# alexfrom0815/IR-BPP

Measured on AMD Instinct MI355X. Metric: env steps/sec (placements/sec) across N parallel bins, higher is better.
Workload: dtype f64

## Files before the change

### irbpp_amd/csrc/irbpp_kernels.hip

```cpp
#include <hip/hip_runtime.h>
#include <math.h>
#include <stdint.h>

#include "contours_device.h"
#include "irbpp_device.h"
#include "../../include/irbpp.h"

#ifndef IRBPP_PASS
#define IRBPP_PASS 1
#endif

#undef IRBPP_HERE
#undef IRBPP_PASS_NS
#if IRBPP_PASS == 1
#define IRBPP_HERE ::irbpp::
#elif IRBPP_PASS == 2
#define IRBPP_HERE ::irbpp::wg512::
#define IRBPP_PASS_NS wg512
#else
#define IRBPP_HERE ::irbpp::wg128::
#define IRBPP_PASS_NS wg128
#endif

namespace irbpp {
// ... 1295 lines not shown
                    khi[l] = ah; klo[l] = al; kps[l] = (uint16_t)ap;
                }
            }
            const int j_next = j > 1 ? (j >> 1) : k;
            if (j >= 128 || j_next >= 128 || (j == 1 && k == npad)) __syncthreads();
            else IRBPP_WAVE_SYNC();
        }
    for (int r = tid; r < want; r += BLOCK) out[r] = sel[kps[r]];
    __syncthreads();
}

#ifdef IRBPP_AB_EMIT_ACCOUNT
#define IRBPP_EMIT_STAMP(k) do { if (io.phase_cycles && threadIdx.x == 0) io.phase_cycles[(size_t)b * PHASE_ROW + (k)] = (long long)clock64(); } while (0)
#else
#define IRBPP_EMIT_STAMP(k) do {} while (0)
#endif
__device__ inline void emit_observation(const Params& P, const State& S, const StepIO& io, const Lds& L, int b, int item,
                                        int nvalid, float* obs, const double* zsrc, const uint32_t* gvalid, uint32_t amap) {
    const int tid = threadIdx.x;
    const int R = P.R, AC = P.AC, Ax = P.Ax, Ay = P.Ay;
    const int X = fdiv(tid, Ay, P.mg_ay), Y = tid - X * Ay;
    const int prev_rows = io.obs_rows != nullptr ? io.obs_rows[b] : -1;
    if (tid == 0) ((unsigned long long*)L.redd)[7] = ~0ull;
    uint32_t* keys = (uint32_t*)L.scratch;
    uint32_t* okey = keys + R * AC;
    uint32_t* hist = (uint32_t*)L.img;
    int n = 0;
    if (tid < 64) {
        const int lane = tid, cx = lane & 15;
        for (int r0 = 0; r0 < R; r0 += 4) {
            const int r = r0 + (lane >> 4);
            uint32_t col = 0u;
            if (r < R && cx < Ay) {
                const uint32_t* const vrow = L.vmask + ((amap >> (4 * r)) & 15u) * 16;
#pragma unroll
                for (int cy = 0; cy < 16; ++cy) col |= ((vrow[cy] >> cx) & 1u) << cy;
                col &= (1u << Ax) - 1u;
            }
            const int cnt = __popc(col), incl = wave_inclusive_sum(cnt);
            int at = n + incl - cnt;
            while (col != 0u) {
                const int cy = __ffs((int)col) - 1;
                col &= col - 1u;
                keys[at++] = ((uint32_t)r << 16) | ((uint32_t)cy << 8) | (uint32_t)cx;
            }
            n += __builtin_amdgcn_readlane(incl, 63);
        }
        if (tid == 0) L.redi[34] = n;
    }
    __syncthreads();
    n = L.redi[34];
    IRBPP_EMIT_STAMP(11);
    int nrows;
    bool fallback = false;
    const uint32_t* rows;
    if (n > 0 && n <= P.S) {
        nrows = n;
        rows = keys;
    } else if (n > P.S) {
        select_smallest(P, L, zsrc, nullptr, n, P.S, [&](int e) { return keys[e]; }, okey, keys, hist);
        nrows = P.S;
        rows = okey;
        __syncthreads();
    } else {
        fallback = true;
        const int total_cells = R * AC;
        const int want = total_cells < P.S ? total_cells : P.S;
        auto cell_key = [&](int e) {
            const int r = fdiv(e, AC, P.mg_ac), c = e - r * AC, x = fdiv(c, Ay, P.mg_ay);
            return ((uint32_t)r << 16) | ((uint32_t)x << 8) | (uint32_t)(c - x * Ay);
        };
        if (nvalid == 0) {
            for (int e = tid; e < want; e += BLOCK) okey[e] = cell_key(e);
            __syncthreads();
        } else {
            select_smallest(P, L, zsrc, gvalid, total_cells, want, cell_key, okey, keys, hist);
        }
        nrows = total_cells < P.S ? total_cells : P.S;
        rows = okey;
        __syncthreads();
    }

    IRBPP_EMIT_STAMP(12);
    int write_rows = P.S;
    if (io.obs_rows != nullptr) {
        if (prev_rows >= 0) write_rows = prev_rows > nrows ? prev_rows : nrows;
        if (tid == 0) io.obs_rows[b] = nrows;
    }
    float best = INFINITY;
    int bi = 0x7fffffff;
    for (int rep = 0; rep < IRBPP_REPS(3); ++rep)
    for (int row = tid; row < write_rows; row += BLOCK) {
        float v0 = 0.0f, v1 = 0.0f, v2 = 0.0f, v3 = 0.0f, v4 = 0.0f;
        if (row < nrows) {
            const uint32_t k = rows[row];
            float rv;
            if (fallback) rv = (float)((gvalid[(k >> 16) * 16 + ((k >> 8) & 255u)] >> (k & 255u)) & 1u);
            else rv = (float)zsrc[(k >> 16) * AC + ((k >> 8) & 255u) * Ay + (k & 255u)];
            v0 = (float)(k >> 16);
            v1 = (float)((k >> 8) & 255u);
            v2 = (float)(k & 255u);
            v3 = fallback ? (float)P.bin_z : rv;
            v4 = fallback ? rv : 1.0f;
            S.cand[(size_t)b * P.S + row] = k;
            if (!fallback && rv < best) { best = rv; bi = row; }
        }
        float* const o = obs + 5 * row;
        o[0] = v0; o[1] = v1; o[2] = v2; o[3] = v3; o[4] = v4;
    }
    IRBPP_EMIT_STAMP(13);
    if (tid == 0) {
        S.bs[b].cur_item = item;
        S.bs[b].nvalid = nvalid;
        S.bs[b].nrows = nrows;
    }
    if (io.auto_action != nullptr) {
        {
#define IRBPP_ARGMIN_STEP(CTRL, ROWS)                                                                                          \
            {                                                                                                                  \
                const float ob = __int_as_float(__builtin_amdgcn_update_dpp(__float_as_int(best), __float_as_int(best), CTRL, ROWS, 0xF, false)); \
                const int oi = __builtin_amdgcn_update_dpp(bi, bi, CTRL, ROWS, 0xF, false);                                     \
                if (ob < best || (ob == best && oi < bi)) { best = ob; bi = oi; }                                               \
            }
            IRBPP_ARGMIN_STEP(0x111, 0xF) IRBPP_ARGMIN_STEP(0x112, 0xF) IRBPP_ARGMIN_STEP(0x114, 0xF) IRBPP_ARGMIN_STEP(0x118, 0xF)
            IRBPP_ARGMIN_STEP(0x142, 0xA) IRBPP_ARGMIN_STEP(0x143, 0xC)
#undef IRBPP_ARGMIN_STEP
        }
        if ((tid & 63) == 63) {
            const uint32_t fb = (uint32_t)__float_as_int(best + 0.0f);
            const uint32_t su = fb ^ ((fb >> 31) != 0u ? 0xFFFFFFFFu : 0x80000000u);
            atomicMin((unsigned long long*)L.redd + 7, ((unsigned long long)su << 32) | (uint32_t)bi);
        }
        __syncthreads();
        if (tid == 0) {
            const int won = (int)(uint32_t)(((const unsigned long long*)L.redd)[7] & 0xFFFFFFFFull);
            io.auto_action[b] = won == 0x7fffffff ? 0 : won;
        }
    }
    stamp(io, b, 4);
}

#endif
template <int IPT>
__device__ inline void split_handover(const Params& P, const State& S, const Lds& L, int b, int slot, int item, int nvalid) {
    const int tid = threadIdx.x;
    const KernArgsPtr ka = cold_args();
    constexpr int IMGS = IPT * (BLOCK / 16);
    constexpr int CLIST = CONTOUR_CLIST;
    uint16_t* const rows = (uint16_t*)L.scratch;
    uint16_t* const cwords = rows + IMGS * 16;
    uint16_t* const clist = L.clist;
    {
        uint32_t* gb = ka->S.w_valid + (size_t)b * P.R * 16;
        for (int rep = 0; rep < IRBPP_REPS(14); ++rep)
#pragma unroll 1
        for (int i = tid; i < P.R * 16; i += BLOCK) gb[i] = L.vbits[i];
        __syncthreads();
    }
    int ntasks = 0;
    for (int rep = 0; rep < IRBPP_REPS(9); ++rep) { if (rep) __syncthreads(); ntasks = IRBPP_HERE contour_tasks(P, L); }
    int ncand = 0, niso = 0;
    uint32_t* gi = (uint32_t*)(ka->S.w_img + (size_t)b * P.wimg * 16);
    uint8_t* gr = ka->S.w_imgrot + (size_t)b * P.wimg;
    const int xcd = (int)(__builtin_amdgcn_s_getreg((31 << 11) | 20) & (NXCD - 1));
    for (int base = 0; base < ntasks; base += IMGS) {
        int batch_total = 0;
        for (int rep = 0; rep < IRBPP_REPS(9); ++rep) {
            IRBPP_HERE contour_images<IPT>(P, L, rows, base, false);
            batch_total = IRBPP_HERE contour_candidates<IPT>(P, L, rows, base, ntasks, cwords);
        }
        niso += batch_total >> 16;
        batch_total &= 0xFFFF;
        const int nb = ntasks - base < IMGS ? ntasks - base : IMGS;
        const uint32_t* lr = (const uint32_t*)rows;
        for (int rep = 0; rep < IRBPP_REPS(14); ++rep) {
#pragma unroll 1
        for (int i = tid; i < nb * 8; i += BLOCK) gi[(size_t)base * 8 + i] = lr[i];
#pragma unroll 1
        for (int i = tid; i < nb; i += BLOCK) gr[base + i] = (uint8_t)(L.tasklist[base + i] >> 8);
        }
        const int nsub = batch_total <= CLIST ? 1 : IMGS;
        for (int sub = 0; sub < nsub; ++sub) {
            int total = 0;
            for (int rep = 0; rep < IRBPP_REPS(10); ++rep) total = IRBPP_HERE contour_list<IPT>(L, rows, clist, base, ntasks, nsub, sub, cwords);
            if (tid == 0) {
                int at = -1, seg = xcd;
                if (total > 0) {
                    for (int k = 0; k < NXCD && at < 0; ++k) {
                        seg = (xcd + k) & (NXCD - 1);
                        const int got = atomicAdd(ka->S.w_total + seg * XCD_STRIDE, total);
                        if (got + total <= P.seg_cap) at = got;
                        else atomicSub(ka->S.w_total + seg * XCD_STRIDE, total);
                    }
                    if (at < 0) raise_error(S, IRBPP_DEVERR_CAPACITY);
                }
                L.redi[11] = at;
                L.redi[12] = seg;
            }
            __syncthreads();
            if (L.redi[11] >= 0) {
                uint2* flat = ka->S.w_cand + (size_t)L.redi[12] * P.seg_cap + L.redi[11];
#pragma unroll 1
                for (int i = tid; i < total; i += BLOCK) {
                    const uint32_t e = clist[i];
                    flat[i] = make_uint2((uint32_t)b, ((uint32_t)(base + (e & 127u)) << 8) | (((e >> 11) & 15u) << 4) | ((e >> 7) & 15u));
                }
            }
            ncand += total;
        }
        __syncthreads();
    }
    uint32_t* gv = ka->S.w_vmask + (size_t)b * P.R * 16;
    for (int rep = 0; rep < IRBPP_REPS(14); ++rep)
#pragma unroll 1
    for (int i = tid; i < P.R * 16; i += BLOCK) gv[i] = L.vmask[i];
    if (tid == 0) {
        int32_t* m = ka->S.w_meta + (size_t)b * WMETA;
        m[0] = ntasks;
        m[1] = ncand;
        m[2] = nvalid;
        m[3] = item;
        m[5] = (int32_t)alias_map(L, P.R, item);
        int heavy = 0;
        const int turn = ka->io.heavy_turn;
        if (turn >= 0 && ncand + niso >= P.heavy_thr) {
            int32_t* hv = ka->S.w_heavy + (size_t)turn * (XCD_STRIDE + P.heavy_cap);
            const int pos = atomicAdd(hv, 1);
            if (pos < P.heavy_cap) { hv[XCD_STRIDE + pos] = b; heavy = 1; }
        }
        m[4] = heavy;
    }
}

#if IRBPP_PASS == 1
template <bool HEAVY_FIRST, int SPEC>
__device__ __forceinline__ void emit_body(const Params& P_run, const Tables& T, const State& S, const StepIO& io, const int mode, unsigned char* smem) {
    Params P_spec;
    const Params& P = SPEC == 0 ? P_run : (P_spec = specialise<SPEC>(P_run), P_spec);
    Lds L = {};
    L.vmask = (uint32_t*)(smem + P.e_vmask);
    L.redd = (double*)(smem + P.e_red);
    L.redi = (int*)(L.redd + 8);
    L.img = (uint16_t*)(smem + P.e_hist);
    L.scratch = smem + P.e_keys;
    const bool some = mode == MODE_RESET && io.bin_list != nullptr;
    const int tid = threadIdx.x;
    if (blockIdx.x == 0 && tid < NXCD) { S.w_total[tid * XCD_STRIDE] = 0; S.w_nround[tid * XCD_STRIDE] = 0; }
    if (blockIdx.x == 0 && tid == 0 && io.err_out != nullptr) *io.err_out = *S.err;
#ifdef IRBPP_AB_EMIT_ACCOUNT
    const long long t_entry = (long long)clock64();
#endif
    int slot = (int)blockIdx.x + io.block_off, b = 0;
    bool mapped = false;
    if constexpr (HEAVY_FIRST) {
        const int hg = io.heavy_turn >= 0 ? P.heavy_cap : 0;
        if ((int)blockIdx.x < hg) {
            const int32_t* hv = S.w_heavy + (size_t)io.heavy_turn * (XCD_STRIDE + P.heavy_cap);
            if (blockIdx.x == 0 && tid == 0) S.w_heavy[(size_t)(io.heavy_turn ^ 1) * (XCD_STRIDE + P.heavy_cap)] = 0;
            int cnt = hv[0];
            cnt = cnt < P.heavy_cap ? cnt : P.heavy_cap;
            if ((int)blockIdx.x >= cnt) return;
            b = hv[XCD_STRIDE + blockIdx.x];
            slot = b;
            mapped = true;
        } else {
            slot -= hg;
        }
    }
    if (!mapped) {
        b = ((mode == MODE_STEP || mode == MODE_CANDS) && io.use_order) ? S.order[slot] : some ? io.bin_list[slot] : slot;
        if constexpr (HEAVY_FIRST)
            if (io.heavy_turn >= 0 && b >= 0 && b < P.N && S.w_meta[(size_t)b * WMETA + 4] != 0) return;
    }
    if (b < 0 || b >= P.N) return;
#ifdef IRBPP_AB_EMIT_ACCOUNT
    if (io.phase_cycles && tid == 0) { io.phase_cycles[(size_t)b * PHASE_ROW + 6] = t_entry; io.phase_cycles[(size_t)b * PHASE_ROW + 7] = (long long)clock64(); }
#endif
    float* obs = io.obs + (size_t)(some ? slot : b) * io.obs_stride;
    const uint32_t* gv = S.w_vmask + (size_t)b * P.R * 16;
#pragma unroll 1
    for (int i = tid; i < P.R * 16; i += BLOCK) L.vmask[i] = gv[i];
    const int nvalid = S.w_meta[(size_t)b * WMETA + 2], item = S.w_meta[(size_t)b * WMETA + 3];
    const uint32_t amap = (uint32_t)S.w_meta[(size_t)b * WMETA + 5];
    __syncthreads();
    stamp(io, b, 3);
    emit_observation(P, S, io, L, b, item, nvalid, obs, S.w_posz + (size_t)b * P.R * P.AC, S.w_valid + (size_t)b * P.R * 16, amap);
    IRBPP_EMIT_STAMP(14);
}
#define IRBPP_EMIT_KERNEL(NAME, HF, SPEC)                                                                                \
    extern "C" __global__ void __launch_bounds__(BLOCK) __attribute__((amdgpu_waves_per_eu(8, 8)))                      \
    NAME(const Params P, const Tables T, const State S, const StepIO io, const int mode) {                              \
        extern __shared__ __attribute__((aligned(16))) unsigned char smem[];                                            \
        emit_body<HF, SPEC>(P, T, S, io, mode, smem);                                                                   \
    }
IRBPP_EMIT_KERNEL(irbpp_emit_kernel, true, 0)
#ifndef IRBPP_NO_SPEC
IRBPP_EMIT_KERNEL(irbpp_emit_kernel_s1, true, 1)
IRBPP_EMIT_KERNEL(irbpp_emit_kernel_s2, true, 2)
IRBPP_EMIT_KERNEL(irbpp_emit_kernel_s3, true, 3)
IRBPP_EMIT_KERNEL(irbpp_emit_kernel_s4, true, 4)
IRBPP_EMIT_KERNEL(irbpp_emit_kernel_s5, true, 5)
#endif

template <int SPEC>
__device__ __forceinline__ void emit_wave_body(const Params& P_run, const Tables& T, const State& S, const StepIO& io, const int mode,
                                               unsigned char* smem) {
    Params P_spec;
    const Params& P = SPEC == 0 ? P_run : (P_spec = specialise<SPEC>(P_run), P_spec);
    int* const need = (int*)(smem + P.e_need);
    const int tid = threadIdx.x, lane = tid & 63, wave = __builtin_amdgcn_readfirstlane(tid >> 6);
    const int R = P.R, AC = P.AC, Ax = P.Ax, Ay = P.Ay;
    const bool some = mode == MODE_RESET && io.bin_list != nullptr;
    if (blockIdx.x == 0 && tid < NXCD) { S.w_total[tid * XCD_STRIDE] = 0; S.w_nround[tid * XCD_STRIDE] = 0; }
    if (blockIdx.x == 0 && tid == 0 && io.err_out != nullptr) *io.err_out = *S.err;
    const int local = (int)blockIdx.x * WAVES + wave;
    const int slot = local + io.block_off;
    int b = -1;
    if (local < io.n_slots) b = ((mode == MODE_STEP || mode == MODE_CANDS) && io.use_order) ? S.order[slot] : some ? io.bin_list[slot] : slot;
    if (b >= P.N) b = -1;
    b = __builtin_amdgcn_readfirstlane(b);
    if (lane == 0) need[wave] = -1;
    if (b >= 0) {
        uint32_t* const vm = (uint32_t*)(smem + wave * P.ew_bytes);
        uint32_t* const keys = vm + R * 16;
        const uint32_t* gv = S.w_vmask + (size_t)b * R * 16;
        for (int i = lane; i < R * 16; i += 64) vm[i] = gv[i];
        const int nvalid = S.w_meta[(size_t)b * WMETA + 2], item = S.w_meta[(size_t)b * WMETA + 3];
        const uint32_t amap = (uint32_t)S.w_meta[(size_t)b * WMETA + 5];
        const int prev_rows = io.obs_rows != nullptr ? io.obs_rows[b] : -1;
        float* const obs = io.obs + (size_t)(some ? slot : b) * io.obs_stride;
        const double* const zsrc = S.w_posz + (size_t)b * R * AC;
        const uint32_t* const gvalid = S.w_valid + (size_t)b * R * 16;
        stamp(io, b, 3, lane == 0);
        IRBPP_WAVE_SYNC();
        const int cx = lane & 15;
        auto column = [&](int r) {
            uint32_t col = 0u;
            if (r < R && cx < Ay) {
                const uint32_t* const vrow = vm + ((amap >> (4 * r)) & 15u) * 16;
#pragma unroll
                for (int cy = 0; cy < 16; ++cy) col |= ((vrow[cy] >> cx) & 1u) << cy;
                col &= (1u << Ax) - 1u;
            }
            return col;
        };
        int n = 0;
#pragma unroll 1
        for (int r0 = 0; r0 < R; r0 += 4) n += __builtin_amdgcn_readlane(wave_inclusive_sum(__popc(column(r0 + (lane >> 4)))), 63);
        if (n > P.S || (n == 0 && nvalid > 0)) {
            if (lane == 0) need[wave] = b;
        } else {
            int at0 = 0;
#pragma unroll 1
            for (int r0 = 0; r0 < R; r0 += 4) {
                const int r = r0 + (lane >> 4);
                uint32_t col = column(r);
                const int cnt = __popc(col), incl = wave_inclusive_sum(cnt);
                int at = at0 + incl - cnt;
                while (col != 0u) {
                    const int cy = __ffs((int)col) - 1;
                    col &= col - 1u;
                    keys[at++] = ((uint32_t)r << 16) | ((uint32_t)cy << 8) | (uint32_t)cx;
                }
                at0 += __builtin_amdgcn_readlane(incl, 63);
            }
            IRBPP_WAVE_SYNC();
            const bool fallback = n == 0;
            const int total_cells = R * AC;
            const int nrows = fallback ? (total_cells < P.S ? total_cells : P.S) : n;
            int write_rows = P.S;
            if (io.obs_rows != nullptr) {
                if (prev_rows >= 0) write_rows = prev_rows > nrows ? prev_rows : nrows;
                if (lane == 0) io.obs_rows[b] = nrows;
            }
            float best = INFINITY;
            int bi = 0x7fffffff;
            for (int row = lane; row < write_rows; row += 64) {
                float v0 = 0.0f, v1 = 0.0f, v2 = 0.0f, v3 = 0.0f, v4 = 0.0f;
                if (row < nrows) {
                    uint32_t k;
                    if (fallback) {
                        const int r = fdiv(row, AC, P.mg_ac), c = row - r * AC, x = fdiv(c, Ay, P.mg_ay);
                        k = ((uint32_t)r << 16) | ((uint32_t)x << 8) | (uint32_t)(c - x * Ay);
                    } else {
                        k = keys[row];
                    }
                    float rv;
                    if (fallback) rv = (float)((gvalid[(k >> 16) * 16 + ((k >> 8) & 255u)] >> (k & 255u)) & 1u);
                    else rv = (float)zsrc[(k >> 16) * AC + ((k >> 8) & 255u) * Ay + (k & 255u)];
                    v0 = (float)(k >> 16);
                    v1 = (float)((k >> 8) & 255u);
                    v2 = (float)(k & 255u);
                    v3 = fallback ? (float)P.bin_z : rv;
                    v4 = fallback ? rv : 1.0f;
                    S.cand[(size_t)b * P.S + row] = k;
                    if (!fallback && rv < best) { best = rv; bi = row; }
                }
                float* const o = obs + 5 * row;
                o[0] = v0; o[1] = v1; o[2] = v2; o[3] = v3; o[4] = v4;
            }
            if (lane == 0) {
                S.bs[b].cur_item = item;
                S.bs[b].nvalid = nvalid;
                S.bs[b].nrows = nrows;
            }
            if (io.auto_action != nullptr) {
#define IRBPP_ARGMIN_STEP(CTRL, ROWS)                                                                                          \
                {                                                                                                              \
                    const float ob = __int_as_float(__builtin_amdgcn_update_dpp(__float_as_int(best), __float_as_int(best), CTRL, ROWS, 0xF, false)); \
                    const int oi = __builtin_amdgcn_update_dpp(bi, bi, CTRL, ROWS, 0xF, false);                                 \
                    if (ob < best || (ob == best && oi < bi)) { best = ob; bi = oi; }                                           \
                }
                IRBPP_ARGMIN_STEP(0x111, 0xF) IRBPP_ARGMIN_STEP(0x112, 0xF) IRBPP_ARGMIN_STEP(0x114, 0xF) IRBPP_ARGMIN_STEP(0x118, 0xF)
                IRBPP_ARGMIN_STEP(0x142, 0xA) IRBPP_ARGMIN_STEP(0x143, 0xC)
#undef IRBPP_ARGMIN_STEP
                if (lane == 63) io.auto_action[b] = bi == 0x7fffffff ? 0 : bi;
            }
            stamp(io, b, 4, lane == 0);
        }
    }
    __syncthreads();
    if ((need[0] & need[1] & need[2] & need[3]) == -1) return;
    Lds L = {};
    L.vmask = (uint32_t*)(smem + P.e_vmask);
    L.redd = (double*)(smem + P.e_red);
    L.redi = (int*)(L.redd + 8);
    L.img = (uint16_t*)(smem + P.e_hist);
    L.scratch = smem + P.e_keys;
#pragma unroll 1
    for (int w = 0; w < WAVES; ++w) {
        const int bw = __builtin_amdgcn_readfirstlane(need[w]);
        if (bw < 0) continue;
        const int slot_w = (int)blockIdx.x * WAVES + w + io.block_off;
        float* const obs = io.obs + (size_t)(some ? slot_w : bw) * io.obs_stride;
        const uint32_t* gv = S.w_vmask + (size_t)bw * R * 16;
        __syncthreads();
#pragma unroll 1
        for (int i = tid; i < R * 16; i += BLOCK) L.vmask[i] = gv[i];
        const int nvalid = S.w_meta[(size_t)bw * WMETA + 2], item = S.w_meta[(size_t)bw * WMETA + 3];
        const uint32_t amap_w = (uint32_t)S.w_meta[(size_t)bw * WMETA + 5];
        __syncthreads();
        stamp(io, bw, 3);
        emit_observation(P, S, io, L, bw, item, nvalid, obs, S.w_posz + (size_t)bw * R * AC, S.w_valid + (size_t)bw * R * 16, amap_w);
    }
}
#define IRBPP_EMIT_WAVE_KERNEL(NAME, SPEC)                                                                                  \
    extern "C" __global__ void __launch_bounds__(BLOCK) __attribute__((amdgpu_waves_per_eu(8, 8)))                      \
    NAME(const Params P, const Tables T, const State S, const StepIO io, const int mode) {                              \
        extern __shared__ __attribute__((aligned(16))) unsigned char smem[];                                            \
        emit_wave_body<SPEC>(P, T, S, io, mode, smem);                                                                  \
    }
IRBPP_EMIT_WAVE_KERNEL(irbpp_emit_wave_kernel, 0)
#ifndef IRBPP_NO_SPEC
IRBPP_EMIT_WAVE_KERNEL(irbpp_emit_wave_kernel_s1, 1)
IRBPP_EMIT_WAVE_KERNEL(irbpp_emit_wave_kernel_s2, 2)
IRBPP_EMIT_WAVE_KERNEL(irbpp_emit_wave_kernel_s5, 5)
#endif

#ifndef IRBPP_TRACE_SHORT
#define IRBPP_TRACE_SHORT 0
#endif
constexpr int TRACE_P = IRBPP_TRACE_P;
constexpr int TRACE_CAP = 128;
constexpr int TRACE_LDS_CAP = 56, TRACE_SLOT = TRACE_LDS_CAP + 4;
constexpr int TRACE_SPILL = TRACE_CAP - TRACE_LDS_CAP;
constexpr int TRACE_SHORT = IRBPP_TRACE_SHORT;
static_assert(TRACE_CAP <= 64 * TRACE_P, "a border must fit one polygon round");
static_assert(ROUND_POINTS == 64 * TRACE_P, "a round record holds one polygon round");
constexpr int TRACE_BIG = 768;
constexpr int TRACE_FSTRIDE = FRAME_WORDS;
static_assert(TRACE_FSTRIDE % 2 == 1 && (TRACE_SLOT / 4) % 2 == 1 && TRACE_SLOT % 4 == 0, "odd dword strides in LDS");
constexpr int TRACE_BIG_BYTES = 6 * TRACE_BIG + 64;
constexpr int TRACE_WAVE_BYTES = TRACE_BIG_BYTES + 64 * TRACE_SPILL;
template <int TRACE_CPW>
__device__ __forceinline__ void trace_body(const Params& P, const State& S, long long* prof) {
    constexpr int SLOT = TRACE_SLOT, CAP = TRACE_CAP, LCAP = TRACE_LDS_CAP, PP = TRACE_P;
    __shared__ __attribute__((aligned(16))) uint8_t slots[TRACE_CPW * SLOT];
    __shared__ __attribute__((aligned(16))) uint32_t sfr[TRACE_CPW * TRACE_FSTRIDE];
    __shared__ uint32_t dps[64 * PP];
    __shared__ uint8_t dpscratch[64 * PP];
    const int lane = threadIdx.x;
    const int seg_cap = P.seg_cap;
    int seg_n[NXCD], seg_first[NXCD + 1];
    seg_first[0] = 0;
#pragma unroll
    for (int s = 0; s < NXCD; ++s) {
        const int n = S.w_total[s * XCD_STRIDE];
        seg_n[s] = n < seg_cap ? n : seg_cap;
        seg_first[s + 1] = seg_first[s] + (seg_n[s] + TRACE_CPW - 1) / TRACE_CPW;
    }
    for (int chunk = blockIdx.x; chunk < seg_first[NXCD]; chunk += gridDim.x) {
        const long long t_start = prof ? (long long)clock64() : 0;
        int seg = 0;
#pragma unroll
        for (int s = 1; s < NXCD; ++s) seg += chunk >= seg_first[s] ? 1 : 0;
        int first_chunk = 0, count = 0;
#pragma unroll
        for (int s = 0; s < NXCD; ++s) if (s == seg) { first_chunk = seg_first[s]; count = seg_n[s]; }
        const int gi = (chunk - first_chunk) * TRACE_CPW + lane;
        const bool have = lane < TRACE_CPW && gi < count;
        const size_t g = (size_t)seg * seg_cap + gi;
        int my_n = 0, rk = 0, x0 = 0, y0 = 0;
        uint32_t* const fr = sfr + (lane < TRACE_CPW ? lane : 0) * TRACE_FSTRIDE;
        uint8_t* const my_slot = slots + (lane < TRACE_CPW ? lane : 0) * SLOT;
        uint8_t* const wave_spill = S.w_big + (size_t)blockIdx.x * TRACE_WAVE_BYTES + TRACE_BIG_BYTES;
        if (have) {
            const uint2 ce = S.w_cand[g];
            const uint32_t e = ce.y;
            const int b = (int)ce.x, img = (int)((e >> 8) & 511u);
            x0 = e & 15u;
            y0 = (e >> 4) & 15u;
            rk = b * P.R + (int)S.w_imgrot[(size_t)b * P.wimg + img];
            const uint4* gi = (const uint4*)(S.w_img + ((size_t)b * P.wimg + img) * 16);
            const uint4 v0 = gi[0], v1 = gi[1];
            const uint32_t w[8] = {v0.x, v0.y, v0.z, v0.w, v1.x, v1.y, v1.z, v1.w};
            uint32_t r[16], c[16];
#pragma unroll
            for (int q = 0; q < 8; ++q) {
                r[2 * q] = c[2 * q] = w[q] & 0xFFFFu;
                r[2 * q + 1] = c[2 * q + 1] = w[q] >> 16;
            }
            transpose16(c);
            frames_store(fr, r, c);
        }
        const long long t_staged = prof ? (long long)clock64() : 0;
        {
            const int n = trace_border_fast(fr, x0, y0, my_slot, LCAP, have, wave_spill + lane * TRACE_SPILL, TRACE_SPILL);
            if (n < 0) { if (lane == 0) atomicOr(S.err, IRBPP_DEVERR_TRACE_GUARD); }
            else my_n = n;
        }
        {
            unsigned long long big = __ballot(my_n > CAP);
            while (big != 0ull) {
                const int l0 = __ffsll((long long)big) - 1;
                big &= big - 1ull;
                if (lane == l0) {
                    uint8_t* gsc = S.w_big + (size_t)blockIdx.x * TRACE_WAVE_BYTES;
                    SlotMem m;
                    m.pts = gsc; m.dst = gsc + TRACE_BIG; m.stk = (uint32_t*)(gsc + 2 * TRACE_BIG); m.cap = TRACE_BIG; m.cap_stk = TRACE_BIG;
                    uint16_t* im = (uint16_t*)(gsc + 6 * TRACE_BIG);
                    for (int q = 0; q < 16; ++q) { im[q] = (uint16_t)frame_raw_row(fr, q); im[16 + q] = (uint16_t)frame_raw_col(fr, q); }
                    if (contour_vertices(im, im + 16, x0, y0, m, S.w_vmask + (size_t)rk * 16) != 0)
                        atomicOr(S.err, IRBPP_DEVERR_TRACE_GUARD);
                    my_n = 0;
                }
            }
        }
        const bool spilled = __ballot(my_n > LCAP) != 0ull;
        if (spilled) {
            __builtin_amdgcn_fence(__ATOMIC_RELEASE, "workgroup");
            __builtin_amdgcn_fence(__ATOMIC_ACQUIRE, "workgroup");
        }
        const long long t_traced = prof ? (long long)clock64() : 0;
        auto next_round = [&](int cls, int left, int& wn, int& excl, int& base) -> unsigned long long {
            wn = (cls == 0 ? left <= TRACE_SHORT : true) ? left : 0;
            const int incl = wave_inclusive_sum(wn);
            excl = incl - wn;
            if (__builtin_amdgcn_readlane(incl, 63) == 0) return 0ull;
            const unsigned long long todo = __ballot(wn > 0);
            base = __builtin_amdgcn_readlane(excl, __ffsll((long long)todo) - 1);
            return __ballot(wn > 0 && incl - base <= 64 * PP);
        };
        int n_rounds = 0;
        {
            int left = my_n;
            for (int cls = 0; cls < 2; ++cls)
                for (;;) {
                    int wn, excl, base = 0;
                    const unsigned long long sel = next_round(cls, left, wn, excl, base);
                    if (sel == 0ull) break;
                    if ((sel >> lane) & 1ull) left = 0;
                    ++n_rounds;
                }
        }
        const int round_cap = P.round_cap;
        const int xcd = (int)(__builtin_amdgcn_s_getreg((31 << 11) | 20) & (NXCD - 1));
        int at = 0;
        if (n_rounds > 0) {
            if (lane == 0) at = atomicAdd(S.w_nround + xcd * XCD_STRIDE, n_rounds);
            at = __builtin_amdgcn_readfirstlane(at);
        }
        const bool inline_dp = at + n_rounds > round_cap;
        uint8_t* const rec0 = S.w_round + ((size_t)xcd * round_cap + at) * ROUND_BYTES;
        int left = my_n, n_dp = 0;
        for (int cls = 0; cls < 2; ++cls)
        for (;;) {
            int wn, excl, base = 0;
            const unsigned long long sel = next_round(cls, left, wn, excl, base);
            if (sel == 0ull) break;
#pragma unroll
            for (int u = 0; u < PP; ++u) dps[u * 64 + lane] = 0u;
            IRBPP_WAVE_SYNC();
            if ((sel >> lane) & 1ull) dps[excl - base] = (uint32_t)lane + 1u;
            IRBPP_WAVE_SYNC();
            int mark[PP];
#pragma unroll
            for (int u = 0; u < PP; ++u) mark[u] = (int)dps[u * 64 + lane];
            IRBPP_WAVE_SYNC();
            bool live[PP];
            int pv[PP], jj[PP], nn[PP], sbq[PP], prk[PP];
            const uint8_t* pts[PP];
            int carry = 0;
#pragma unroll
            for (int u = 0; u < PP; ++u) {
                const int run = imax(wave_inclusive_max(mark[u]), carry);
                carry = __builtin_amdgcn_readlane(run, 63);
                const int owner = run - 1;
                const int on = owner >= 0 ? owner : 0;
                const int ns = __shfl(wn | ((excl - base) << 8), on);
                nn[u] = ns & 255;
                sbq[u] = ns >> 8;
                prk[u] = __shfl(rk, on);
                live[u] = owner >= 0 && u * 64 + lane < sbq[u] + nn[u];
                pts[u] = slots + on * SLOT;
                jj[u] = u * 64 + lane - sbq[u];
                if (!live[u]) { nn[u] = 1; sbq[u] = 0; jj[u] = 0; }
                pv[u] = live[u] ? (int)pts[u][jj[u] < LCAP ? jj[u] : LCAP] : 0;
                if (spilled && live[u] && jj[u] >= LCAP) pv[u] = (int)wave_spill[on * TRACE_SPILL + jj[u] - LCAP];
            }
            if (inline_dp) {
                approx_convex_segmented<PP>(lane, live, pv, jj, nn, sbq, pts, prk, dps, dpscratch, S.w_vmask);
            } else {
                uint8_t* const rec = rec0 + (size_t)n_dp * ROUND_BYTES;
#pragma unroll
                for (int u = 0; u < PP; ++u) {
                    const int q = u * 64 + lane;
                    rec[q] = (uint8_t)pv[u];
                    rec[64 * PP + q] = (uint8_t)(live[u] ? nn[u] : 0);
                    rec[2 * 64 * PP + q] = (uint8_t)sbq[u];
                    ((uint32_t*)(rec + 3 * 64 * PP))[q] = (uint32_t)prk[u];
                }
            }
            if ((sel >> lane) & 1ull) left = 0;
            ++n_dp;
        }
        if (inline_dp && n_rounds > 0 && at < round_cap) {
            const int lim = at + n_rounds < round_cap ? n_rounds : round_cap - at;
            for (int i = 0; i < lim; ++i)
#pragma unroll
                for (int u = 0; u < PP; ++u) rec0[(size_t)i * ROUND_BYTES + 64 * PP + u * 64 + lane] = 0;
        }
#if defined(IRBPP_AB_POLY_ACCOUNT) || defined(IRBPP_AB_EMIT_ACCOUNT)
        if (false) {
#else
        if (prof && lane == 0) {
#endif
            const int b0 = (int)S.w_cand[(size_t)seg * seg_cap + (size_t)(chunk - first_chunk) * TRACE_CPW].x;
            long long* row = prof + (size_t)b0 * PHASE_ROW;
            const long long t_end = (long long)clock64();
            row[11] = t_end - t_start;
            row[12] = t_staged - t_start;
            row[13] = t_traced - t_staged;
            row[14] = t_end - t_traced;
            row[15] = 1 | ((long long)n_dp << 20) | ((long long)(count - (chunk - first_chunk) * TRACE_CPW < TRACE_CPW ? count - (chunk - first_chunk) * TRACE_CPW : TRACE_CPW) << 40);
        }
        IRBPP_WAVE_SYNC();
    }
}

constexpr int TRACE_REFILL_BATCH = 128, TRACE_REFILL_THR = 32;
template <int BATCH, int THR>
__device__ __forceinline__ void trace_refill_body(const Params& P, const State& S, long long* prof) {
    constexpr int SLOT = TRACE_SLOT, CAP = TRACE_CAP, LCAP = TRACE_LDS_CAP, PP = TRACE_P, NCE = BATCH / 64;
    static_assert(BATCH % 64 == 0 && NCE >= 1 && NCE <= 4, "a batch is a whole number of wave-wide candidate loads");
    __shared__ __attribute__((aligned(16))) uint8_t slots[64 * SLOT];
    __shared__ __attribute__((aligned(16))) uint32_t sfr[64 * TRACE_FSTRIDE];
    __shared__ uint32_t dps[64 * PP];
    __shared__ uint8_t dpscratch[64 * PP];
    const int lane = threadIdx.x;
    const int seg_cap = P.seg_cap;
    int seg_n[NXCD], seg_first[NXCD + 1];
    seg_first[0] = 0;
#pragma unroll
    for (int s = 0; s < NXCD; ++s) {
        const int n = S.w_total[s * XCD_STRIDE];
        seg_n[s] = n < seg_cap ? n : seg_cap;
        seg_first[s + 1] = seg_first[s] + (seg_n[s] + BATCH - 1) / BATCH;
    }
    uint32_t* const fr = sfr + lane * TRACE_FSTRIDE;
    uint8_t* const my_slot = slots + lane * SLOT;
    uint8_t* const wave_spill = S.w_big + (size_t)blockIdx.x * TRACE_WAVE_BYTES + TRACE_BIG_BYTES;
    uint8_t* const my_spill = wave_spill + lane * TRACE_SPILL;
    IRBPP_WALK_TABLES(WT)
    const int round_cap = P.round_cap;
    const int xcd = (int)(__builtin_amdgcn_s_getreg((31 << 11) | 20) & (NXCD - 1));
    for (int chunk = blockIdx.x; chunk < seg_first[NXCD]; chunk += gridDim.x) {
        const long long t_start = prof ? (long long)clock64() : 0;
        int seg = 0;
#pragma unroll
        for (int s = 1; s < NXCD; ++s) seg += chunk >= seg_first[s] ? 1 : 0;
        int first_chunk = 0, count = 0;
#pragma unroll
        for (int s = 0; s < NXCD; ++s) if (s == seg) { first_chunk = seg_first[s]; count = seg_n[s]; }
        const int gi0 = (chunk - first_chunk) * BATCH;
        const int nb = count - gi0 < BATCH ? count - gi0 : BATCH;
        const uint2* const cl = S.w_cand + (size_t)seg * seg_cap + gi0;
        uint2 ce[NCE];
#pragma unroll
        for (int u = 0; u < NCE; ++u) ce[u] = u * 64 + lane < nb ? cl[u * 64 + lane] : make_uint2(0u, 0u);
        Walk w;
        w.pos = w.n = w.result = w.pos0 = w.pos1 = 0;
        w.nb16 = w.k2 = w.prev = w.s_close = w.run = 0u;
        int rk = 0, x0 = 0, y0 = 0, nxt = 0, n_dp_total = 0, refills = 0;
        uint2 pf_e = make_uint2(0u, 0u);
        uint4 pf0 = make_uint4(0u, 0u, 0u, 0u), pf1 = pf0;
        uint32_t pf_rot = 0u;
        auto prefetch = [&]() {
            const int c = nxt + lane;
            uint2 e = make_uint2(0u, 0u);
#pragma unroll
            for (int u = 0; u < NCE; ++u) {
                const uint32_t ex = (uint32_t)__shfl((int)ce[u].x, c & 63), ey = (uint32_t)__shfl((int)ce[u].y, c & 63);
                if ((c >> 6) == u) e = make_uint2(ex, ey);
            }
            pf_e = e;
            if (c < nb) {
                const size_t at = (size_t)e.x * P.wimg + ((e.y >> 8) & 511u);
                pf_rot = S.w_imgrot[at];
                const uint4* gi = (const uint4*)(S.w_img + at * 16);
                pf0 = gi[0];
                pf1 = gi[1];
            }
        };
        auto flush = [&]() {
            int my_n = w.run == 0u ? w.result : 0;
            w.result = w.run == 0u ? 0 : w.result;
            if (__ballot(my_n != 0) == 0ull) return;
            {
                unsigned long long big = __ballot(my_n > CAP);
                while (big != 0ull) {
                    const int l0 = __ffsll((long long)big) - 1;
                    big &= big - 1ull;
                    if (lane == l0) {
                        uint8_t* gsc = S.w_big + (size_t)blockIdx.x * TRACE_WAVE_BYTES;
                        SlotMem m;
                        m.pts = gsc; m.dst = gsc + TRACE_BIG; m.stk = (uint32_t*)(gsc + 2 * TRACE_BIG); m.cap = TRACE_BIG; m.cap_stk = TRACE_BIG;
                        uint16_t* im = (uint16_t*)(gsc + 6 * TRACE_BIG);
                        for (int q = 0; q < 16; ++q) { im[q] = (uint16_t)frame_raw_row(fr, q); im[16 + q] = (uint16_t)frame_raw_col(fr, q); }
                        if (contour_vertices(im, im + 16, x0, y0, m, S.w_vmask + (size_t)rk * 16) != 0)
                            atomicOr(S.err, IRBPP_DEVERR_TRACE_GUARD);
                        my_n = 0;
                    }
                }
            }
            const bool spilled = __ballot(my_n > LCAP) != 0ull;
            if (spilled) {
                __builtin_amdgcn_fence(__ATOMIC_RELEASE, "workgroup");
// ... 1122 lines not shown
```

Measured before the change: 71.87 million.

## Single-pass candidate key scan, split emit loops, outline rare fallback path

The wave emit path now counts and writes candidate keys in one pass over the rows, capping writes at P.S, instead of scanning the valid mask twice. The per-row output loop is split into separate non-fallback, fallback and zero-padding loops with strength-reduced pointers, which removes per-iteration branches. The rare block-wide fallback (emit_observation) moves into a noinline function that reloads its arguments through cold_args(), aimed at lowering register pressure in the hot kernel. In exchange there is a call overhead on the rare path, and keys may be partly written before the overflow check sends the bin to the fallback.

```diff
diff --git a/irbpp_amd/csrc/irbpp_kernels.hip b/irbpp_amd/csrc/irbpp_kernels.hip
--- a/irbpp_amd/csrc/irbpp_kernels.hip
+++ b/irbpp_amd/csrc/irbpp_kernels.hip
@@ -1621,6 +1621,38 @@
 IRBPP_EMIT_KERNEL(irbpp_emit_kernel_s5, true, 5)
 #endif
 
+__device__ __noinline__ void emit_wave_rare(const KernArgsPtr ka_v, unsigned char* smem, const int* need, const bool some) {
+    const uint64_t ka_u = (uint64_t)ka_v;
+    const KernArgsPtr ka = (KernArgsPtr)(((uint64_t)(uint32_t)__builtin_amdgcn_readfirstlane((int)(ka_u >> 32)) << 32) |
+                                         (uint32_t)__builtin_amdgcn_readfirstlane((int)(uint32_t)ka_u));
+    const Params& P = *(const Params*)&ka->P;
+    const State& S = *(const State*)&ka->S;
+    const StepIO& io = *(const StepIO*)&ka->io;
+    const int tid = threadIdx.x, R = P.R, AC = P.AC;
+    Lds L = {};
+    L.vmask = (uint32_t*)(smem + P.e_vmask);
+    L.redd = (double*)(smem + P.e_red);
+    L.redi = (int*)(L.redd + 8);
+    L.img = (uint16_t*)(smem + P.e_hist);
+    L.scratch = smem + P.e_keys;
+#pragma unroll 1
+    for (int w = 0; w < WAVES; ++w) {
+        const int bw = __builtin_amdgcn_readfirstlane(need[w]);
+        if (bw < 0) continue;
+        const int slot_w = (int)blockIdx.x * WAVES + w + io.block_off;
+        float* const obs = io.obs + (size_t)(some ? slot_w : bw) * io.obs_stride;
+        const uint32_t* gv = S.w_vmask + (size_t)bw * R * 16;
+        __syncthreads();
+#pragma unroll 1
+        for (int i = tid; i < R * 16; i += BLOCK) L.vmask[i] = gv[i];
+        const int nvalid = S.w_meta[(size_t)bw * WMETA + 2], item = S.w_meta[(size_t)bw * WMETA + 3];
+        const uint32_t amap_w = (uint32_t)S.w_meta[(size_t)bw * WMETA + 5];
+        __syncthreads();
+        stamp(io, bw, 3);
+        emit_observation(P, S, io, L, bw, item, nvalid, obs, S.w_posz + (size_t)bw * R * AC, S.w_valid + (size_t)bw * R * 16, amap_w);
+    }
+}
+
 template <int SPEC>
 __device__ __forceinline__ void emit_wave_body(const Params& P_run, const Tables& T, const State& S, const StepIO& io, const int mode,
                                                unsigned char* smem) {
@@ -1653,7 +1685,10 @@
         stamp(io, b, 3, lane == 0);
         IRBPP_WAVE_SYNC();
         const int cx = lane & 15;
-        auto column = [&](int r) {
+        int n = 0;
+#pragma unroll 1
+        for (int r0 = 0; r0 < R; r0 += 4) {
+            const int r = r0 + (lane >> 4);
             uint32_t col = 0u;
             if (r < R && cx < Ay) {
                 const uint32_t* const vrow = vm + ((amap >> (4 * r)) & 15u) * 16;
@@ -1661,28 +1696,19 @@
                 for (int cy = 0; cy < 16; ++cy) col |= ((vrow[cy] >> cx) & 1u) << cy;
                 col &= (1u << Ax) - 1u;
             }
-            return col;
-        };
-        int n = 0;
-#pragma unroll 1
-        for (int r0 = 0; r0 < R; r0 += 4) n += __builtin_amdgcn_readlane(wave_inclusive_sum(__popc(column(r0 + (lane >> 4)))), 63);
+            const int cnt = __popc(col), incl = wave_inclusive_sum(cnt);
+            const int end = n + incl < P.S ? n + incl : P.S;
+            const uint32_t base = ((uint32_t)r << 16) | (uint32_t)cx;
+            for (int at = n + incl - cnt; at < end; ++at) {
+                const int cy = __ffs((int)col) - 1;
+                col &= col - 1u;
+                keys[at] = base | ((uint32_t)cy << 8);
+            }
+            n += __builtin_amdgcn_readlane(incl, 63);
+        }
         if (n > P.S || (n == 0 && nvalid > 0)) {
             if (lane == 0) need[wave] = b;
         } else {
-            int at0 = 0;
-#pragma unroll 1
-            for (int r0 = 0; r0 < R; r0 += 4) {
-                const int r = r0 + (lane >> 4);
-                uint32_t col = column(r);
-                const int cnt = __popc(col), incl = wave_inclusive_sum(cnt);
-                int at = at0 + incl - cnt;
-                while (col != 0u) {
-                    const int cy = __ffs((int)col) - 1;
-                    col &= col - 1u;
-                    keys[at++] = ((uint32_t)r << 16) | ((uint32_t)cy << 8) | (uint32_t)cx;
-                }
-                at0 += __builtin_amdgcn_readlane(incl, 63);
-            }
             IRBPP_WAVE_SYNC();
             const bool fallback = n == 0;
             const int total_cells = R * AC;
@@ -1694,30 +1720,29 @@
             }
             float best = INFINITY;
             int bi = 0x7fffffff;
-            for (int row = lane; row < write_rows; row += 64) {
-                float v0 = 0.0f, v1 = 0.0f, v2 = 0.0f, v3 = 0.0f, v4 = 0.0f;
-                if (row < nrows) {
-                    uint32_t k;
-                    if (fallback) {
-                        const int r = fdiv(row, AC, P.mg_ac), c = row - r * AC, x = fdiv(c, Ay, P.mg_ay);
-                        k = ((uint32_t)r << 16) | ((uint32_t)x << 8) | (uint32_t)(c - x * Ay);
-                    } else {
-                        k = keys[row];
-                    }
-                    float rv;
-                    if (fallback) rv = (float)((gvalid[(k >> 16) * 16 + ((k >> 8) & 255u)] >> (k & 255u)) & 1u);
-                    else rv = (float)zsrc[(k >> 16) * AC + ((k >> 8) & 255u) * Ay + (k & 255u)];
-                    v0 = (float)(k >> 16);
-                    v1 = (float)((k >> 8) & 255u);
-                    v2 = (float)(k & 255u);
-                    v3 = fallback ? (float)P.bin_z : rv;
-                    v4 = fallback ? rv : 1.0f;
-                    S.cand[(size_t)b * P.S + row] = k;
-                    if (!fallback && rv < best) { best = rv; bi = row; }
+            int row = lane;
+            float* o = obs + 5 * lane;
+            uint32_t* cd = S.cand + (size_t)b * P.S + lane;
+            if (!fallback) {
+                const uint32_t* kp = keys + lane;
+                for (; row < nrows; row += 64, o += 5 * 64, cd += 64, kp += 64) {
+                    const uint32_t k = *kp;
+                    const uint32_t kr = k >> 16, kx = (k >> 8) & 255u, ky = k & 255u;
+                    const float rv = (float)zsrc[kr * (uint32_t)AC + kx * (uint32_t)Ay + ky];
+                    *cd = k;
+                    if (rv < best) { best = rv; bi = row; }
+                    o[0] = (float)kr; o[1] = (float)kx; o[2] = (float)ky; o[3] = rv; o[4] = 1.0f;
                 }
-                float* const o = obs + 5 * row;
-                o[0] = v0; o[1] = v1; o[2] = v2; o[3] = v3; o[4] = v4;
-            }
+            } else {
+                const float hz = (float)P.bin_z;
+                for (; row < nrows; row += 64, o += 5 * 64, cd += 64) {
+                    const int r = fdiv(row, AC, P.mg_ac), c = row - r * AC, x = fdiv(c, Ay, P.mg_ay), y = c - x * Ay;
+                    const float rv = (float)((gvalid[r * 16 + x] >> y) & 1u);
+                    *cd = ((uint32_t)r << 16) | ((uint32_t)x << 8) | (uint32_t)y;
+                    o[0] = (float)r; o[1] = (float)x; o[2] = (float)y; o[3] = hz; o[4] = rv;
+                }
+            }
+            for (; row < write_rows; row += 64, o += 5 * 64) { o[0] = 0.0f; o[1] = 0.0f; o[2] = 0.0f; o[3] = 0.0f; o[4] = 0.0f; }
             if (lane == 0) {
                 S.bs[b].cur_item = item;
                 S.bs[b].nvalid = nvalid;
@@ -1740,28 +1765,7 @@
     }
     __syncthreads();
     if ((need[0] & need[1] & need[2] & need[3]) == -1) return;
-    Lds L = {};
-    L.vmask = (uint32_t*)(smem + P.e_vmask);
-    L.redd = (double*)(smem + P.e_red);
-    L.redi = (int*)(L.redd + 8);
-    L.img = (uint16_t*)(smem + P.e_hist);
-    L.scratch = smem + P.e_keys;
-#pragma unroll 1
-    for (int w = 0; w < WAVES; ++w) {
-        const int bw = __builtin_amdgcn_readfirstlane(need[w]);
-        if (bw < 0) continue;
-        const int slot_w = (int)blockIdx.x * WAVES + w + io.block_off;
-        float* const obs = io.obs + (size_t)(some ? slot_w : bw) * io.obs_stride;
-        const uint32_t* gv = S.w_vmask + (size_t)bw * R * 16;
-        __syncthreads();
-#pragma unroll 1
-        for (int i = tid; i < R * 16; i += BLOCK) L.vmask[i] = gv[i];
-        const int nvalid = S.w_meta[(size_t)bw * WMETA + 2], item = S.w_meta[(size_t)bw * WMETA + 3];
-        const uint32_t amap_w = (uint32_t)S.w_meta[(size_t)bw * WMETA + 5];
-        __syncthreads();
-        stamp(io, bw, 3);
-        emit_observation(P, S, io, L, bw, item, nvalid, obs, S.w_posz + (size_t)bw * R * AC, S.w_valid + (size_t)bw * R * 16, amap_w);
-    }
+    emit_wave_rare(cold_args(), smem, need, some);
 }
 #define IRBPP_EMIT_WAVE_KERNEL(NAME, SPEC)                                                                                  \
     extern "C" __global__ void __launch_bounds__(BLOCK) __attribute__((amdgpu_waves_per_eu(8, 8)))                      \
```

New measurement: 71.81 million. No clear change (-0.1%).
